# szcompressor/SZ3

Measured on AMD Instinct MI355X. Metric: compression throughput GB/s + ratio at fixed abs errBound, 512^3 f32, higher is better.
Workload: dtype f32; 1 GPU; C2: 3D float32 512x512x512 synthetic field per GPU, Lorenzo predictor, abs errBound=0.001, device-resident in -> device-resident Huffman payload; parallelism=slab1, algo=HIP_LORENZO(16), exchange=none (one rank)

## Files before the change

include/sz3hip_debug.h:

```cpp
#ifndef SZ3HIP_DEBUG_H
#define SZ3HIP_DEBUG_H

enum sz3hip_dbg {
    SZ3HIP_DBG_CB_COMPACT_IN_WG = 1,
    SZ3HIP_DBG_K1_LAB_NO_HIST = 1,
    SZ3HIP_DBG_DEC_MULTI_SYM = 2,
    SZ3HIP_DBG_K1_NO_CODE_STORES = 2,
    SZ3HIP_DBG_BLKDEC_FORCE_RETRY = 4,
    SZ3HIP_DBG_K1_V4_NO_STENCIL = 4,
    SZ3HIP_DBG_K1_NO_Q16 = 8,
    SZ3HIP_DBG_BLKDEC_LOCAL_EXPANDED = 16,
    SZ3HIP_DBG_K1_V4_NO_PREFETCH = 16,
    SZ3HIP_DBG_PACK_LAB_NO_STORES = 16,
    SZ3HIP_DBG_K1_NO_MARCH = 32,
    SZ3HIP_DBG_K1_NO_NARROW = 64,
    SZ3HIP_DBG_INTERP_NO_VEC = 128,
    SZ3HIP_DBG_K1_NO_WIDTH_SPEC = 256,
    SZ3HIP_DBG_DEC_NO_FUSED_X = 512,
    SZ3HIP_DBG_PACK_LAB_ONE_UNIT = 512,
    SZ3HIP_DBG_CB_ONE_CLASS = 1024,
    SZ3HIP_DBG_K1_NO_FUSED = 2048,
    SZ3HIP_DBG_BLK_RANK_3_LAUNCHES = 2048,
    SZ3HIP_DBG_BLK_SIDE_8_LAUNCHES = 2048,
    SZ3HIP_DBG_K1_NO_XCD_ORDER = 4096,
// ... 15 lines not shown
    SZ3HIP_DBG_K1_Q16_PLAIN_STORES = 8388608,
    SZ3HIP_DBG_K1_NO_DEFER_FOLD = 16777216,
    SZ3HIP_DBG_PACK_NO_SEG_BITS = 33554432,
    SZ3HIP_DBG_BLK_FIT_TILES = 67108864,
    SZ3HIP_DBG_BLK_1D_WAVE_PER_BLOCK = 134217728,
    SZ3HIP_DBG_CTX_NO_PUBLISH_ZERO = 268435456,
    SZ3HIP_DBG_INTERP_HANDOVER_IN_PLACE = 536870912,
    SZ3HIP_DBG_DEC_CARRY_PASS = 536870912,
    SZ3HIP_DBG_BLK_NO_EXIT = 1073741824,
    SZ3HIP_DBG_BLK_NO_SELECT = -2147483647 - 1
};

enum sz3hip_dbg2 {
    SZ3HIP_DBG2_PACK_SCAN_LAUNCH = 1,
    SZ3HIP_DBG2_REQUEST_BY_LEVEL = 2,
    SZ3HIP_DBG2_MAP_PLAIN_STORES = 4
};

#endif
```

sz3_amd/__init__.py:

```python
import contextlib
import ctypes as C
import enum
import os

import numpy as np

_HERE = os.path.dirname(os.path.abspath(__file__))
LIB_PATH = os.environ.get("SZ3HIP_LIB") or os.path.join(_HERE, "libsz3hip.so")

EB_ABS, EB_REL, EB_PSNR, EB_L2NORM, EB_ABS_AND_REL, EB_ABS_OR_REL = range(6)
ALGO_LORENZO_REG, ALGO_INTERP_LORENZO, ALGO_INTERP, ALGO_NOPRED, ALGO_LOSSLESS = range(5)
ALGO_HIP_LORENZO = 16
ALGO_HIP_INTERP = 17
INTERP_ALGO_LINEAR, INTERP_ALGO_CUBIC = 0, 1
SZ_FLOAT, SZ_DOUBLE = 0, 1


class Dbg(enum.IntFlag):
    CB_COMPACT_IN_WG = 1
    K1_LAB_NO_HIST = 1
    DEC_MULTI_SYM = 2
    K1_NO_CODE_STORES = 2
    BLKDEC_FORCE_RETRY = 4
    K1_V4_NO_STENCIL = 4
# ... 31 lines not shown
    K1_NO_DEFER_FOLD = 16777216
    PACK_NO_SEG_BITS = 33554432
    BLK_FIT_TILES = 67108864
    BLK_1D_WAVE_PER_BLOCK = 134217728
    CTX_NO_PUBLISH_ZERO = 268435456
    INTERP_HANDOVER_IN_PLACE = 536870912
    DEC_CARRY_PASS = 536870912
    BLK_NO_EXIT = 1073741824
    BLK_NO_SELECT = 2147483648


class Dbg2(enum.IntFlag):
    PACK_SCAN_LAUNCH = 1
    REQUEST_BY_LEVEL = 2
    MAP_PLAIN_STORES = 4


class SZ3HipError(RuntimeError):
    def __init__(self, code, msg):
        super().__init__("sz3hip error %d: %s" % (code, msg))
        self.code = code


class _CConfig(C.Structure):
    _fields_ = [
        ("N", C.c_int32), ("dims", C.c_uint64 * 4), ("num", C.c_uint64),
        ("cmprAlgo", C.c_uint8), ("errorBoundMode", C.c_uint8),
        ("absErrorBound", C.c_double), ("relErrorBound", C.c_double),
        ("psnrErrorBound", C.c_double), ("l2normErrorBound", C.c_double),
        ("openmp", C.c_uint8), ("quantbinCnt", C.c_int32), ("blockSize", C.c_int32),
# ... 1447 lines not shown
```

sz3_amd/csrc/sz3hip_kernels.h:

```cpp
#ifndef SZ3HIP_KERNELS_H
#define SZ3HIP_KERNELS_H
#include <hip/hip_runtime.h>
#include <stdint.h>
#include "sz3hip_format.h"
#include "../../include/sz3hip_debug.h"

struct szk_lattice {
    double recip, two_eb, eb;
    float recip_f, two_eb_f, eb_lo_f;
};
static inline szk_lattice szk_make_lattice(double eb) {
    szk_lattice l;
    l.eb = eb;
    l.two_eb = 2.0 * eb;
    l.recip = 1.0 / l.two_eb;
    l.recip_f = (float)l.recip;
    l.two_eb_f = (float)l.two_eb;
    float e = (float)eb;
    if ((double)e > eb) e = __builtin_nextafterf(e, 0.0f);
    l.eb_lo_f = e;
    return l;
}

#define SZK_K1_GRID 2048u
// ... 4 lines not shown
    uint32_t pack_wide;
    uint64_t n_samples;
    uint64_t n_total;
    uint32_t allow;
};

struct szk_cb_info;
#define SZK_SAMP_UNITS 1024u
#define SZK_SAMP_ROLES 128u
#define SZK_SAMP_MIN_ELEMS (1ull << 22)
#define SZK_SAMP_SEEN_LEN 16u
#define SZK_SAMP_WORDS 512u
#define SZK_SAMP_TICKET 320u
#define SZK_SAMP_LENS 384u
#define SZK_SAMP_READY 448u
struct szk_samp {
    uint32_t *words;
    uint32_t *enc;
    uint8_t *lens;
    szk_cb_info *info;
};
struct szk_k1_params {
    uint64_t d[4];
    szk_lattice lat;
    uint32_t radius;
    uint32_t dbg;
    szk_mode mode;
    uint64_t out_cap;
    uint64_t *hist;
    uint32_t *hist_partial;
// ... 14 lines not shown
    uint32_t *q16_flag;
    int defer_fold;
    uint32_t fold_rows;
    int range_kept;
    int fuse;
    int fused;
    const uint32_t *fuse_enc;
    const szk_cb_info *fuse_info;
    uint32_t *fuse_slots;
    uint64_t fuse_cap_words;
    uint32_t *seg_base;
    uint32_t *fuse_flag;
    uint32_t fuse_geom[4];
    szk_samp samp;
    int samp_in_launch;
};

struct szk_cb_info {
    uint32_t n_symbols, max_len, sym_min, sym_count;
    uint32_t win_lo, reserved;
    uint32_t esc_sym, pad0;
    uint64_t ts[12];
    uint32_t first_code[SZH_MAX_LEN + 2];
};
#define SZK_CB_DBG_ONE_CLASS 1u
#define SZK_CB_DBG_SERIAL_MERGE 2u
struct szk_cb_params {
    uint32_t *enc;
    uint8_t *lens;
    uint64_t *keys;
// ... 461 lines not shown
```

sz3_amd/csrc/sz3hip_kernels.hip:

```cpp
#include <hip/hip_runtime.h>
#include <cstddef>
#include <stdint.h>
#include <type_traits>
#include <mutex>
#include <utility>
#include <vector>
#include "sz3hip_format.h"
#include "sz3hip_kernels.h"

#include "sz3hip_devutil.h"

template <typename T>
__global__ __launch_bounds__(256) void k_minmax(const T *__restrict__ in, uint64_t n, double *partial) {
    double mn = INFINITY, mx = -INFINITY;
    bool has_nan = false;
    for (uint64_t i = (uint64_t)blockIdx.x * blockDim.x + threadIdx.x; i < n; i += (uint64_t)gridDim.x * blockDim.x) {
        double v = (double)in[i];
        if (v < mn) mn = v;
        if (v > mx) mx = v;
        has_nan |= (v != v);
    }
    (void)has_nan;
#pragma unroll
    for (int d = WAVE / 2; d > 0; d >>= 1) {
// ... 815 lines not shown
    uint16_t *seg_bits;
    uint64_t *oq_idx;
    OQV *oq_val;
    uint32_t oq_n;
    int lane;
    const uint32_t *s_enc;
    uint32_t *stage;
    uint32_t *slot;
    uint32_t slot_base;
    uint32_t slot_w;
    uint32_t st_cnt;
    uint32_t *seg_base;
    const uint32_t *samp_words;
    uint32_t *s_have;
    uint32_t have_len;
};
#define FUSE_STAGE_WORDS(TY) ((TY) * 128 + 32 + 8)
static inline uint32_t fuse_slot_words(uint32_t ty, uint64_t d1, uint64_t d2) {
    return (uint32_t)((d1 < ty ? d1 : ty) * 128u * (d2 < MARCH_TZ ? d2 : MARCH_TZ) + 32u);
}
template <typename T>
__device__ __forceinline__ void narrow_oq_flush(NarrowCtx<T> &c) {
    c.oq_n = (uint32_t)__builtin_amdgcn_readfirstlane((int)c.oq_n);
    if (c.oq_n == 0) return;
    const szk_k1_params &p = *c.p;
    const unsigned long long act = __ballot(1);
    const uint32_t nact = (uint32_t)__popcll(act), rank = (uint32_t)__popcll(act & ((1ull << c.lane) - 1ull));
    unsigned long long base = 0;
    if (rank == 0) base = atomicAdd((unsigned long long *)p.n_vout, (unsigned long long)c.oq_n);
    const uint32_t blo = (uint32_t)__builtin_amdgcn_readfirstlane((int)(uint32_t)base);
// ... 43 lines not shown
                c.oq_val[slot] = bits;
            }
            c.oq_n += (uint32_t)__popcll(vm);
        }
    }
    {
        const uint32_t cnt = (uint32_t)__popc(tmask & 15u);
        const unsigned long long b0 = __ballot(cnt & 1u), b1 = __ballot(cnt & 2u), b2 = __ballot(cnt & 4u), any = b0 | b1 | b2;
        if (any && c.lane == __ffsll((long long)any) - 1)
            hist_add_ranged(p.hist, p.range, 0u, (unsigned long long)(__popcll(b0) + 2 * __popcll(b1) + 4 * __popcll(b2)));
    }
}
template <typename T> __device__ __forceinline__ bool samp_take(const T *__restrict__ in, const szk_lattice &latp, uint32_t d0, uint32_t d1, uint32_t d2, uint32_t *words, uint32_t role, uint32_t *s_h);
__device__ __forceinline__ void samp_book(const szk_samp &sp, uint32_t radius, uint8_t *pool);
#define SAMP_POOL_BYTES (SZK_CB_SMALL_SYMS * 28 + 256)
template <typename T, typename PUT>
__device__ __forceinline__ bool samp_poll(NarrowCtx<T> &c, bool spin, PUT put) {
    volatile uint32_t *s_have = c.s_have;
    const uint32_t wv = (uint32_t)__builtin_amdgcn_readfirstlane((int)(threadIdx.x / WAVE));
    if (wv != 0) {
        uint32_t h = (uint32_t)__builtin_amdgcn_readfirstlane((int)*s_have);
        if (!h) {
            if (!spin) return false;
            do {
                __builtin_amdgcn_s_sleep(16);
                h = (uint32_t)__builtin_amdgcn_readfirstlane((int)*s_have);
            } while (!h);
        }
        __builtin_amdgcn_fence(__ATOMIC_ACQUIRE, "workgroup");
        c.have_len = 1;
// ... 102 lines not shown
#pragma unroll
            for (int r = 0; r <= TY; r++) {
                const uint32_t gy = y0 + (uint32_t)r - 1u;
                R.rok[lw][r] = wok && gy < d1;
                if (R.rok[lw][r]) {
                    const T *row = src + (uint64_t)gy * d0;
                    R.rq[lw][r].load(row + lane_off);
                    if (has_left) R.rl[lw][r] = row[x0 - 1];
                }
            }
        }
    };
    NarrowPlane<T, NW, TY> pa;
    auto work = [&](int zz, NarrowPlane<T, NW, TY> &R, bool fetch_next = false) {
        const uint32_t gz = z0 + (uint32_t)zz;
        if constexpr (FUSE) {
            __builtin_amdgcn_s_waitcnt(0x0F70);
            fuse_flush_lines(c);
        }
#if defined(LAB_MODE) && LAB_MODE == 1
        if (zz >= 0) {
#pragma unroll
            for (int r = 1; r <= TY; r++) {
                if (!R.rok[0][r]) continue;
                uint32_t acc = 0;
#pragma unroll
                for (int lw = 0; lw < NW; lw++)
#pragma unroll
                    for (int i = 0; i < 4; i++) acc += (uint32_t)lat.qbits(R.rq[lw][r].get(i)) + (has_left ? (uint32_t)lat.qbits(R.rl[lw][r]) : 0u);
                if (r == 1 && R.rok[0][0]) acc += (uint32_t)lat.qbits(R.rq[0][0].get(0));
// ... 80 lines not shown
#endif
                    const uint32_t l0 = e0 & 31u, l1 = e1 & 31u, l2 = e2 & 31u, l3 = e3 & 31u;
                    fp01[r - 1] = ((e0 >> 5) << l1) | (e1 >> 5);
                    fp23[r - 1] = ((e2 >> 5) << l3) | (e3 >> 5);
                    const uint32_t l23 = l2 + l3;
                    fl[r - 1] = (l0 + l1 + l23) | (l23 << 8);
                } else {
#ifdef LAB_ABLATE
                if (!(c.p->dbg & SZ3HIP_DBG_K1_NO_CODE_STORES))
#endif
#ifdef LAB_PLAIN_STORE
                *reinterpret_cast<uint32_t *>(c.codes8 + grow + x) = t[0] | (t[1] << 8) | (t[2] << 16) | (t[3] << 24);
#else
                __builtin_nontemporal_store(t[0] | (t[1] << 8) | (t[2] << 16) | (t[3] << 24), reinterpret_cast<uint32_t *>(c.codes8 + grow + x));
#endif
                }
            }
            if (SAMP ? c.have_len != 0u : c.s_len != nullptr) {
                uint32_t b4 = (uint32_t)c.s_len[t[0]] + c.s_len[t[1]] + c.s_len[t[2]] + c.s_len[t[3]];
                if (EDGE) b4 = xok ? b4 : 0u;
                bits_rows[(r - 1) >> 1] |= ((r - 1) & 1) ? b4 << 16 : b4;
            }
            if (__builtin_amdgcn_ballot_w64(rare)) {
                uint32_t tmask = 0, badmask = 0;
#pragma unroll
                for (int i = 0; i < 4; i++) {
                    tmask |= (uint32_t)(rare && t[i] == 255u) << i;
                    badmask |= (uint32_t)(rare && bad[i]) << i;
                }
                narrow_rare<T>(c, grow + x, delta, tmask, badmask);
// ... 86 lines not shown
                const uint32_t ra = y0 + 2u * k, rb = ra + 1u;
                if (lane == 0) {
                    const uint64_t g0 = (uint64_t)w * c.vol + (uint64_t)gz * c.plane + x0;
                    if (ra < d1) c.seg_bits[(g0 + (uint64_t)ra * d0) >> 8] = (uint16_t)(tot & 0xFFFFu);
                    if (2 * k + 1 < TY && rb < d1) c.seg_bits[(g0 + (uint64_t)rb * d0) >> 8] = (uint16_t)(tot >> 16);
                }
            }
        }
    };
    int zz = z0 > 0 ? -1 : 0;
    const int zend = d2 - z0 < (uint32_t)MARCH_TZ ? (int)(d2 - z0) : MARCH_TZ;
    if constexpr (SAMP) {
        uint8_t *const lt = const_cast<uint8_t *>(c.s_len);
        auto put_len = [&](uint32_t b, uint32_t len) { lt[b] = (uint8_t)len; };
        auto catch_up = [&](int zhi) __attribute__((always_inline)) {
            asm volatile("s_waitcnt vmcnt(0)" ::: "memory");
            constexpr int PB = 4;
            for (int p0 = 0; p0 < zhi; p0 += PB) {
                uint32_t cw[PB][TY];
#pragma unroll
                for (int j = 0; j < PB; j++) {
                    const uint64_t gp = (uint64_t)(z0 + (uint32_t)(p0 + j)) * c.plane;
#pragma unroll
                    for (int r = 0; r < TY; r++) {
                        const uint32_t ry = y0 + (uint32_t)r;
                        cw[j][r] = 0;
                        if (p0 + j < zhi && ry < d1 && xok)
                            cw[j][r] = __hip_atomic_load(reinterpret_cast<uint32_t *>(c.codes8 + gp + (uint64_t)ry * d0 + x), __ATOMIC_RELAXED, __HIP_MEMORY_SCOPE_WORKGROUP);
                    }
                }
#pragma unroll
                for (int j = 0; j < PB; j++) {
                    const uint64_t gp = (uint64_t)(z0 + (uint32_t)(p0 + j)) * c.plane;
                    if (p0 + j < zhi)
#pragma unroll
                    for (int k = 0; k < (TY + 1) / 2; k++) {
                        uint32_t packed = 0;
#pragma unroll
                        for (int h = 0; h < 2; h++) {
                            const uint32_t ry = y0 + 2u * k + h;
                            if (2 * k + h < TY && ry < d1 && xok) {
                                const uint32_t wd = cw[j][(2 * k + h) < TY ? 2 * k + h : 0];
                                const uint32_t b4 = (uint32_t)c.s_len[wd & 0xFFu] + c.s_len[(wd >> 8) & 0xFFu] + c.s_len[(wd >> 16) & 0xFFu] + c.s_len[wd >> 24];
// ... 35 lines not shown
        }
    } else if (FUSE) {
        fetch(zz, pa);
        for (; zz < zend; zz++) work(zz, pa, zz + 1 < zend);
    } else {
        for (; zz < zend; zz++) {
            fetch(zz, pa);
            work(zz, pa);
        }
    }
}
template <typename T, int NDIM, int TY, bool FUSE = false, bool SAMP = false>
__device__ __forceinline__ void march_narrow(const T *__restrict__ in, uint16_t *__restrict__ codes, const szk_k1_params &p, uint32_t ntasks,
                                             uint32_t *lh, uint8_t *s_len, uint64_t (*s_oq_idx)[MarchLds<1, false>::OQ],
                                             typename NarrowCtx<T>::OQV (*s_oq_val)[MarchLds<1, false>::OQ],
                                             uint32_t *s_fenc = nullptr, uint32_t *s_fstage = nullptr) {
    const Lattice<T> lat(p.lat);
    NarrowCtx<T> c;
    c.in = in;
    c.codes8 = reinterpret_cast<uint8_t *>(codes);
    c.p = &p;
    c.d0 = (uint32_t)p.d[3];
    c.d1 = (uint32_t)p.d[2];
    c.d2 = (uint32_t)p.d[1];
    c.plane = (uint64_t)c.d1 * c.d0;
    c.vol = c.plane * c.d2;
    c.lh = lh;
    c.lane = lane_id();
    const uint32_t wv = (uint32_t)__builtin_amdgcn_readfirstlane((int)(threadIdx.x / WAVE));
    c.oq_idx = s_oq_idx[wv];
    c.oq_val = s_oq_val[wv];
    c.oq_n = 0;
    const bool acct = SAMP || (!FUSE && p.spec_lens != nullptr && c.d0 % MARCH_TX == 0);
    c.s_len = acct ? s_len : nullptr;
    c.seg_bits = p.seg_bits;
    c.s_enc = s_fenc;
    c.stage = nullptr;
    c.slot = nullptr;
    c.slot_w = c.slot_base = c.st_cnt = 0;
    c.seg_base = p.seg_base;
    c.samp_words = p.samp.words;
    c.s_have = lh + NARROW_BINS * 4;
    c.have_len = 0;
    const uint32_t bid = SAMP ? blockIdx.x - SZK_SAMP_ROLES : blockIdx.x, grid = SAMP ? gridDim.x - SZK_SAMP_ROLES : gridDim.x;
    for (int i = threadIdx.x; i < NARROW_BINS * 4; i += 256) lh[i] = 0;
    if (threadIdx.x == 0) lh[NARROW_BINS * 4] = 0;
    if constexpr (FUSE) {
        const uint32_t ml = p.fuse_info->max_len, blo = p.fuse_info->sym_min, bcnt = p.fuse_info->sym_count;
        const uint32_t b = threadIdx.x;
        const uint32_t sym = b == 255u ? 0u : b + p.radius - 127u;
        s_fenc[b] = (ml <= 16u && sym >= blo && sym - blo < bcnt) ? p.fuse_enc[sym] : 0u;
        if (ml > 16u && blockIdx.x == 0 && threadIdx.x == 0) atomicOr(p.fuse_flag, 1u);
        for (int i = threadIdx.x; i < 4 * FUSE_STAGE_WORDS(TY); i += 256) s_fstage[i] = 0u;
        c.stage = s_fstage + wv * FUSE_STAGE_WORDS(TY);
        if (blockIdx.x == 0 && threadIdx.x == 0) *p.seg_made = 1u;
    }
    if (acct) {
        const uint32_t b = threadIdx.x;
// ... 105 lines not shown
#else
                R.rq[r] = *reinterpret_cast<const float4 *>(row + lane_off);
#endif
                if (has_left) R.rl[r] = row[x0 - 1];
            }
        }
    };
    Q16Plane<TY> pa;
    auto work = [&](int zz, Q16Plane<TY> &R) {
        const uint32_t gz = z0 + (uint32_t)zz;
        uint32_t pd1A = 0, pd1B = 0;
        uint32_t bits_rows[(TY + 1) / 2];
#pragma unroll
        for (int k = 0; k < (TY + 1) / 2; k++) bits_rows[k] = 0;
        float qmax = 0.0f;
#pragma unroll
        for (int r = 0; r <= TY; r++) {
            uint32_t d1A = 0, d1B = 0;
            v2f32 s01 = {0.0f, 0.0f}, s23 = {0.0f, 0.0f}, t01 = magic2, t23 = magic2;
            if (R.rok[r]) {
                const v2f32 v01 = {R.rq[r].x, R.rq[r].y}, v23 = {R.rq[r].z, R.rq[r].w};
                s01 = v01 * recip2;
                s23 = v23 * recip2;
                t01 = s01 + magic2;
                t23 = s23 + magic2;
                uint32_t PA = pk_lo16(__float_as_uint(t01.x), __float_as_uint(t23.x));
                uint32_t PB = pk_lo16(__float_as_uint(t01.y), __float_as_uint(t23.y));
                if (EDGE) {
                    PA = xok ? PA : 0u;
                    PB = xok ? PB : 0u;
// ... 34 lines not shown
                    atomicAdd(reinterpret_cast<uint32_t *>(lds + a0), 1u);
                    atomicAdd(reinterpret_cast<uint32_t *>(lds + a1), 1u);
                    atomicAdd(reinterpret_cast<uint32_t *>(lds + a2), 1u);
                    atomicAdd(reinterpret_cast<uint32_t *>(lds + a3), 1u);
                }
#if defined(LAB_ST) && LAB_ST == 1
                __hip_atomic_store(reinterpret_cast<uint32_t *>(c.codes8 + grow + x), tA | (tB << 8), __ATOMIC_RELAXED, __HIP_MEMORY_SCOPE_SYSTEM);
#elif defined(LAB_ST) && LAB_ST == 2
                *reinterpret_cast<uint32_t *>(c.codes8 + grow + x) = tA | (tB << 8);
#elif defined(LAB_ST) && LAB_ST == 3
                __hip_atomic_store(reinterpret_cast<uint32_t *>(c.codes8 + grow + x), tA | (tB << 8), __ATOMIC_RELAXED, __HIP_MEMORY_SCOPE_AGENT);
#else
                if (c.p->dbg & SZ3HIP_DBG_K1_Q16_PLAIN_STORES) *reinterpret_cast<uint32_t *>(c.codes8 + grow + x) = tA | (tB << 8);
                else __builtin_nontemporal_store(tA | (tB << 8), reinterpret_cast<uint32_t *>(c.codes8 + grow + x));
#endif
            }
            if (SAMP ? c.have_len != 0u : c.s_len != nullptr) {
                uint32_t b4 = (uint32_t)lds[Q16_LEN_OFF + a0] + lds[Q16_LEN_OFF + a1] + lds[Q16_LEN_OFF + a2] + lds[Q16_LEN_OFF + a3];
                if (EDGE) b4 = xok ? b4 : 0u;
                bits_rows[(r - 1) >> 1] |= ((r - 1) & 1) ? b4 << 16 : b4;
            }
            if (__builtin_amdgcn_ballot_w64(rare)) {
                const bool bad[4] = {b0, b1, b2, b3};
                const float sv[4] = {s01.x, s01.y, s23.x, s23.y};
                const uint32_t t[4] = {tA & 0xFFFFu, tB & 0xFFFFu, tA >> 16, tB >> 16};
                const uint32_t delta[4] = {(uint32_t)(int32_t)(int16_t)(sA & 0xFFFFu), (uint32_t)(int32_t)(int16_t)(sB & 0xFFFFu),
                                           (uint32_t)(int32_t)(int16_t)(sA >> 16), (uint32_t)(int32_t)(int16_t)(sB >> 16)};
                uint32_t tmask = 0, badmask = 0;
                bool alien = false;
#pragma unroll
// ... 21 lines not shown
                if (lane == 0) {
                    const uint64_t g0 = (uint64_t)gz * c.plane + x0;
                    if (ra < d1) c.seg_bits[(g0 + (uint64_t)ra * d0) >> 8] = (uint16_t)(tot & 0xFFFFu);
                    if (2 * k + 1 < TY && rb < d1) c.seg_bits[(g0 + (uint64_t)rb * d0) >> 8] = (uint16_t)(tot >> 16);
                }
            }
        }
    };
    int zz = z0 > 0 ? -1 : 0;
    const int zend = d2 - z0 < (uint32_t)MARCH_TZ ? (int)(d2 - z0) : MARCH_TZ;
    auto put_len = [&](uint32_t b, uint32_t len) {
        uint32_t *lt = c.lh + NARROW_BINS * 4 + b * 4u;
        lt[0] = lt[1] = lt[2] = lt[3] = len;
    };
    auto catch_up = [&](int zhi) __attribute__((always_inline)) {
        asm volatile("s_waitcnt vmcnt(0)" ::: "memory");
        constexpr int PB = 4;
        for (int p0 = 0; p0 < zhi; p0 += PB) {
            uint32_t cw[PB][TY];
#pragma unroll
            for (int j = 0; j < PB; j++) {
                const uint64_t gp = (uint64_t)(z0 + (uint32_t)(p0 + j)) * c.plane;
#pragma unroll
                for (int r = 0; r < TY; r++) {
                    const uint32_t ry = y0 + (uint32_t)r;
                    cw[j][r] = 0x80808080u;
                    if (p0 + j < zhi && ry < d1 && xok)
                        cw[j][r] = __hip_atomic_load(reinterpret_cast<uint32_t *>(c.codes8 + gp + (uint64_t)ry * d0 + x), __ATOMIC_RELAXED, __HIP_MEMORY_SCOPE_WORKGROUP);
                }
            }
#pragma unroll
            for (int j = 0; j < PB; j++) {
                const uint64_t gp = (uint64_t)(z0 + (uint32_t)(p0 + j)) * c.plane;
                if (p0 + j < zhi)
#pragma unroll
                for (int k = 0; k < (TY + 1) / 2; k++) {
                    uint32_t packed = 0;
#pragma unroll
                    for (int h = 0; h < 2; h++) {
                        const uint32_t ry = y0 + 2u * k + h;
                        if (2 * k + h < TY && ry < d1 && xok) {
                            const uint32_t w = cw[j][(2 * k + h) < TY ? 2 * k + h : 0];
                            const uint32_t b4 = (uint32_t)lds[Q16_LEN_OFF + (w & 0xFFu) * 16u + c4] + lds[Q16_LEN_OFF + ((w >> 8) & 0xFFu) * 16u + c4] +
// ... 32 lines not shown
        work(zz, pa);
        if (++zz >= zend) break;
        if (zz + 1 < zend) fetch(zz + 1, pa);
        work(zz, pb);
        if (++zz >= zend) break;
    }
#else
    for (; zz < zend; zz++) {
        fetch(zz, pa);
        work(zz, pa);
    }
#endif
}
template <int TY, bool SAMP>
__device__ __forceinline__ void march_narrow16(const float *__restrict__ in, uint16_t *__restrict__ codes, const szk_k1_params &p, uint32_t ntasks,
                                               uint32_t *lh, uint64_t (*s_oq_idx)[MarchLds<1, false>::OQ], uint32_t (*s_oq_val)[MarchLds<1, false>::OQ]) {
    const Lattice<float> lat(p.lat);
    NarrowCtx<float> c;
    c.in = in;
    c.codes8 = reinterpret_cast<uint8_t *>(codes);
    c.p = &p;
    c.d0 = (uint32_t)p.d[3];
    c.d1 = (uint32_t)p.d[2];
    c.d2 = (uint32_t)p.d[1];
    c.plane = (uint64_t)c.d1 * c.d0;
    c.vol = c.plane * c.d2;
    c.lh = lh;
    c.lane = lane_id();
    const uint32_t wv = (uint32_t)__builtin_amdgcn_readfirstlane((int)(threadIdx.x / WAVE));
    c.oq_idx = s_oq_idx[wv];
    c.oq_val = s_oq_val[wv];
    c.oq_n = 0;
    const bool acct = SAMP || (p.spec_lens != nullptr && c.d0 % MARCH_TX == 0);
    c.s_len = acct ? reinterpret_cast<const uint8_t *>(lh) + Q16_LEN_OFF : nullptr;
    c.seg_bits = p.seg_bits;
    c.s_enc = nullptr;
    c.stage = nullptr;
    c.slot = nullptr;
    c.slot_w = c.slot_base = c.st_cnt = 0;
    c.seg_base = p.seg_base;
    c.samp_words = p.samp.words;
    c.s_have = lh + NARROW_BINS * 8;
    c.have_len = 0;
    const uint32_t bid = SAMP ? blockIdx.x - SZK_SAMP_ROLES : blockIdx.x, grid = SAMP ? gridDim.x - SZK_SAMP_ROLES : gridDim.x;
    for (int i = threadIdx.x; i < NARROW_BINS * 4; i += 256) lh[i] = 0;
    if (threadIdx.x == 0) lh[NARROW_BINS * 8] = 0;
    {
        const uint32_t b = threadIdx.x;
        const uint32_t len = (acct && !SAMP) ? p.spec_lens[b == 255u ? 0u : b + p.radius - 127u] : 0u;
#pragma unroll
        for (int k = 0; k < 4; k++) lh[NARROW_BINS * 4 + b * 4 + k] = len;
        if (acct && bid == 0 && threadIdx.x == 0) *p.seg_made = 1u;
    }
    __syncthreads();
    const uint32_t ntx = (c.d0 + MARCH_TX - 1) / MARCH_TX, nty = (c.d1 + TY - 1) / TY;
    const uint32_t per_xcd = grid / 8u;
    const uint32_t wg_seq = grid % 8u == 0 && !(p.dbg & SZ3HIP_DBG_K1_NO_XCD_ORDER) ? (bid % 8u) * per_xcd + bid / 8u : bid;
    const uint32_t nwaves = grid * 4u;
// ... 49 lines not shown
    __shared__ uint64_t s_oq_idx[4][L::OQ];
    __shared__ OQV s_oq_val[4][L::OQ];
    __shared__ uint8_t s_len[256];
    __shared__ uint32_t s_p[4];
    if constexpr (SAMP) {
        static_assert(NDIM == 3, "1-D ... 3-D arrays");
        if (blockIdx.x < SZK_SAMP_ROLES) {
            if (blockIdx.x == 0 && threadIdx.x == 0) p.samp.info->ts[9] = wall_clock64();
            if (samp_take<T>(in, p.lat, (uint32_t)p.d[3], (uint32_t)p.d[2], (uint32_t)p.d[1], p.samp.words, blockIdx.x, lh)) samp_book(p.samp, p.radius, reinterpret_cast<uint8_t *>(lh));
            __syncthreads();
            probe_body<T, NDIM>(in, p, p.mode.n_total, p.mode.probe_big, s_p);
            return;
        }
    }
    probe_body<T, NDIM>(in, p, p.mode.n_total, p.mode.probe_big, s_p);
    march_narrow<T, NDIM, TY, false, SAMP>(in, codes, p, ntasks, lh, s_len, s_oq_idx, s_oq_val);
}
template <int TY, bool SAMP>
__global__ __launch_bounds__(256) void k_lorenzo_quant_march3q(const float *__restrict__ in, uint16_t *__restrict__ codes,
                                                               szk_k1_params p, uint32_t ntasks, uint32_t nrows) {
    using L = MarchLds<1, false>;
    __shared__ uint32_t lh[NARROW_BINS * 8 + 4];
    __shared__ uint64_t s_oq_idx[4][L::OQ];
    __shared__ uint32_t s_oq_val[4][L::OQ];
    __shared__ uint32_t s_p[4];
    if constexpr (SAMP) {
        static_assert(sizeof(lh) >= SAMP_POOL_BYTES && sizeof(lh) >= 4096, "the book's scratch fits the histogram");
        if (blockIdx.x < SZK_SAMP_ROLES) {
            if (blockIdx.x == 0 && threadIdx.x == 0) p.samp.info->ts[9] = wall_clock64();
            if (samp_take<float>(in, p.lat, (uint32_t)p.d[3], (uint32_t)p.d[2], (uint32_t)p.d[1], p.samp.words, blockIdx.x, lh)) samp_book(p.samp, p.radius, reinterpret_cast<uint8_t *>(lh));
            __syncthreads();
            probe_body<float, 3>(in, p, p.mode.n_total, p.mode.probe_big, s_p);
            return;
        }
    }
    probe_body<float, 3>(in, p, p.mode.n_total, p.mode.probe_big, s_p);
    march_narrow16<TY, SAMP>(in, codes, p, ntasks, lh, s_oq_idx, s_oq_val);
}
template <typename T, int NDIM, int TY>
__global__ __launch_bounds__(256) void k_lorenzo_quant_march3f(const T *__restrict__ in, uint16_t *__restrict__ codes,
                                                               szk_k1_params p, uint32_t ntasks, uint32_t nrows) {
    using L = MarchLds<1, false>;
    using OQV = typename std::conditional<sizeof(T) == 4, uint32_t, uint64_t>::type;
    __shared__ uint32_t lh[NARROW_BINS * 4 + 4];
    __shared__ uint64_t s_oq_idx[4][L::OQ];
    __shared__ OQV s_oq_val[4][L::OQ];
    __shared__ uint32_t s_p[4];
    __shared__ uint32_t s_fenc[256];
    __shared__ __align__(16) uint32_t s_fstage[4 * FUSE_STAGE_WORDS(TY)];
    probe_body<T, NDIM>(in, p, p.mode.n_total, p.mode.probe_big, s_p);
    march_narrow<T, NDIM, TY, true>(in, codes, p, ntasks, lh, nullptr, s_oq_idx, s_oq_val, s_fenc, s_fstage);
}
// ... 1187 lines not shown
    if (ln == 0) s_wc[wv] = (uint32_t)__popcll(pm);
    __syncthreads();
    uint32_t a = (uint32_t)__popcll(pm & lower);
    for (uint32_t k = 0; k < wv; k++) a += s_wc[k];
    const uint32_t m = s_wc[0] + s_wc[1] + s_wc[2] + s_wc[3];
    const uint64_t mykey = ((uint64_t)w << 16) | t;
    if (w) keys[a] = mykey;
    __syncthreads();
    uint32_t r = 0;
    if (w)
        for (uint32_t o = 0; o < m; o++) r += keys[o] < mykey;
    __syncthreads();
    if (w) keys[r] = mykey;
    __syncthreads();
    if (t == 0) sp.info->ts[3] = wall_clock64();
    if (t < WAVE) cb_merge_wave32(keys, reinterpret_cast<uint32_t *>(ifreq), pleaf, pint, m);
    __syncthreads();
    if (t == 0) sp.info->ts[4] = wall_clock64();
    for (uint32_t q = t; q + 1 < m; q += CB_THREADS) {
        if (q == m - 2) pint[q] = (uint16_t)q;
        aux[q] = q == m - 2 ? 0 : 1;
    }
    __syncthreads();
    for (uint32_t span = 1; span < m && span < 2 * L; span <<= 1) {
        for (uint32_t q = t; q + 1 < m; q += CB_THREADS) {
            const uint16_t j = pint[q];
            const uint32_t sum = (uint32_t)aux[q] + aux[j];
            aux2[q] = (uint16_t)(sum > 0xFFFFu ? 0xFFFFu : sum);
            pint2[q] = pint[j];
        }
        __syncthreads();
// ... 13 lines not shown
        pleaf[q] = (uint16_t)l;
        atomicAdd(&s_cnt[l], 1u);
    }
    __syncthreads();
    if (s_over) cb_kraft_repair(pleaf, m, s_cnt, L, CB_THREADS, kraft_ws);
    s_l[t] = 0;
    __syncthreads();
    for (uint32_t q = t; q < m; q += CB_THREADS) s_l[(uint32_t)(keys[q] & 0xFFFFu)] = (uint8_t)pleaf[q];
    __syncthreads();
    if (t == 0) sp.info->ts[8] = wall_clock64();
    uint32_t ubits = 0;
    while ((1u << ubits) < n_un) ubits++;
    const uint32_t len = (n_un == 0 || cnt != 0) ? s_l[t] : (uint32_t)s_l[rep] + ubits;
    __syncthreads();
    s_l[t] = (uint8_t)len;
    uint32_t rank = 0;
    for (uint32_t l = 1; l <= SZH_MAX_LEN; l++) {
        const unsigned long long lm = __ballot(len == l);
        if (ln == 0) s_lc[wv][l] = (uint32_t)__popcll(lm);
        if (len == l) rank = (uint32_t)__popcll(lm & lower);
    }
    __syncthreads();
    if (t == 0) {
        uint32_t code = 0, maxl = 0, prev = 0;
        for (uint32_t l = 1; l <= SZH_MAX_LEN; l++) {
            const uint32_t c = s_lc[0][l] + s_lc[1][l] + s_lc[2][l] + s_lc[3][l];
            code = (code + prev) << (l > 1 ? 1 : 0);
            s_first[l] = code;
            prev = c;
            if (c) maxl = l;
        }
        sp.info->n_symbols = 256;
        sp.info->max_len = maxl;
        sp.info->sym_min = lo;
        sp.info->sym_count = 256;
        sp.info->win_lo = lo;
        sp.info->reserved = 0;
        sp.info->esc_sym = esc;
    }
    __syncthreads();
    for (uint32_t k = 0; k < wv; k++) rank += s_lc[k][len];
    const uint32_t e = ((s_first[len] + rank) << 5) | len;
    sp.enc[lo + t] = e;
    sp.lens[lo + t] = (uint8_t)len;
    if (t == 255) sp.enc[0] = e;
    if (t < 64) {
        const uint32_t w4 = (uint32_t)s_l[4 * t] | ((uint32_t)s_l[4 * t + 1] << 8) | ((uint32_t)s_l[4 * t + 2] << 16) | ((uint32_t)s_l[4 * t + 3] << 24);
        __hip_atomic_store(&sp.words[SZK_SAMP_LENS + t], w4, __ATOMIC_RELAXED, __HIP_MEMORY_SCOPE_AGENT);
    }
    asm volatile("s_waitcnt vmcnt(0)" ::: "memory");
    __syncthreads();
    if (t == 0) {
        __hip_atomic_store(&sp.words[SZK_SAMP_READY], 1u, __ATOMIC_RELAXED, __HIP_MEMORY_SCOPE_AGENT);
        sp.info->ts[10] = wall_clock64();
    }
}

template <typename T>
__global__ __launch_bounds__(256) void k_sample(const T *__restrict__ in, szk_k1_params p) {
    __shared__ __align__(16) uint32_t s_pool[(SAMP_POOL_BYTES + 3) / 4 > 1024 ? (SAMP_POOL_BYTES + 3) / 4 : 1024];
    if (!szk_is_narrow(p.mode)) return;
    if (samp_take<T>(in, p.lat, (uint32_t)p.d[3], (uint32_t)p.d[2], (uint32_t)p.d[1], p.samp.words, blockIdx.x, s_pool)) samp_book(p.samp, p.radius, reinterpret_cast<uint8_t *>(s_pool));
}

__global__ __launch_bounds__(1024) void k_cb_compact(const uint64_t *__restrict__ hist, uint64_t *__restrict__ keys, uint16_t *__restrict__ syms,
                                                     uint64_t *__restrict__ part) {
    __shared__ uint32_t s_w[16], s_before, s_oct[48];
    __shared__ unsigned long long s_sum;
    const uint32_t t = threadIdx.x, lane = lane_id(), wv = t / WAVE, w = blockIdx.x;
    if (t == 0) {
// ... 2821 lines not shown
            if (nb > 0x7FFFFFFFull) return -1;
            hipLaunchKernelGGL((k_lorenzo_quant<T, 4, 64, 8, 4>), dim3((uint32_t)nb), dim3(256), 0, s, (const T *)d_in, codes, p);
            break;
    }
    SZK_CHECK_LAUNCH();
    return 0;
}
uint64_t szk_fuse_scratch_words(int ndim, const uint64_t d[4]) {
    if (ndim < 1 || ndim > 3 || d[3] % MARCH_TX != 0 || d[3] >= (1ull << 31) || d[2] >= (1ull << 31) || d[1] >= (1ull << 31)) return 0;
    const uint32_t ty = ndim == 1 ? 1u : (uint32_t)LAB_MTY;
    return march_tasks(d, ty) * fuse_slot_words(ty, d[2], d[1]) + 2;
}
int szk_launch_k1(int dtype, int ndim, const void *d_in, uint16_t *codes, szk_k1_params *p, hipStream_t s) {
    szk_k1_params &pp = *p;
    pp.dbg = (uint32_t)szk_dbg_flags;
    if (szk_dbg_flags & SZ3HIP_DBG_K1_NO_NARROW) pp.mode.allow = 0;
    return dtype == 0 ? launch_k1<float>(ndim, d_in, codes, pp, s) : launch_k1<double>(ndim, d_in, codes, pp, s);
}

int szk_launch_codebook(const uint64_t *d_hist, const szk_cb_params *p, hipStream_t s) {
    const uint32_t nb = p->n_books ? p->n_books : 1;
    szk_cb_params q = *p;
    q.n_books = nb;
    q.dbg = ((szk_dbg_flags & SZ3HIP_DBG_CB_ONE_CLASS) ? SZK_CB_DBG_ONE_CLASS : 0u) | ((szk_dbg_flags & SZ3HIP_DBG_CB_SERIAL_MERGE) ? SZK_CB_DBG_SERIAL_MERGE : 0u);
    if (nb > 1) {
        hipError_t e = hipMemsetAsync(q.range, 0, 16 * nb, s);
        if (e != hipSuccess) return (int)e;
    }
    if (!p->range_ready) hipLaunchKernelGGL(k_hist_range, dim3(SZH_HIST_BINS / 256, nb), dim3(256), 0, s, d_hist, q.range);
    q.keys_ready = nb == 1 && p->part_hint != 0 && !(szk_dbg_flags & SZ3HIP_DBG_CB_COMPACT_IN_WG) ? 1 : 0;
// ... 414 lines not shown
```

Before: 2520 GB/s.

## Stash early-plane codes in LDS for catch-up and publish sample lengths earlier

While the sampled codebook is not yet ready, the first few z-planes of quantized codes are also kept in a per-wave LDS stash. The catch-up pass that later builds histograms or lengths reads those planes from LDS instead of reloading them from global memory, and it skips the full vmcnt wait when every plane it needs is in the stash. Separately, the sample-codebook kernel now publishes code lengths and the ready flag before computing canonical codes, so marching blocks can start using lengths sooner. This costs extra LDS per workgroup, which a static_assert keeps within a five-workgroups-per-CU budget, and adds a per-store branch.

```diff
diff --git a/include/sz3hip_debug.h b/include/sz3hip_debug.h
--- a/include/sz3hip_debug.h
+++ b/include/sz3hip_debug.h
@@ -53,7 +53,8 @@
 enum sz3hip_dbg2 {
     SZ3HIP_DBG2_PACK_SCAN_LAUNCH = 1,
     SZ3HIP_DBG2_REQUEST_BY_LEVEL = 2,
-    SZ3HIP_DBG2_MAP_PLAIN_STORES = 4
+    SZ3HIP_DBG2_MAP_PLAIN_STORES = 4,
+    SZ3HIP_DBG2_K1_NO_STASH = 8
 };
 
 #endif
diff --git a/sz3_amd/__init__.py b/sz3_amd/__init__.py
--- a/sz3_amd/__init__.py
+++ b/sz3_amd/__init__.py
@@ -69,6 +69,7 @@
     PACK_SCAN_LAUNCH = 1
     REQUEST_BY_LEVEL = 2
     MAP_PLAIN_STORES = 4
+    K1_NO_STASH = 8
 
 
 class SZ3HipError(RuntimeError):
diff --git a/sz3_amd/csrc/sz3hip_kernels.h b/sz3_amd/csrc/sz3hip_kernels.h
--- a/sz3_amd/csrc/sz3hip_kernels.h
+++ b/sz3_amd/csrc/sz3hip_kernels.h
@@ -42,6 +42,7 @@
 #define SZK_SAMP_TICKET 320u
 #define SZK_SAMP_LENS 384u
 #define SZK_SAMP_READY 448u
+#define SZK_K1_STASH_PLANES 4
 struct szk_samp {
     uint32_t *words;
     uint32_t *enc;
@@ -86,6 +87,7 @@
     uint32_t fuse_geom[4];
     szk_samp samp;
     int samp_in_launch;
+    uint32_t stash_k;
 };
 
 struct szk_cb_info {
diff --git a/sz3_amd/csrc/sz3hip_kernels.hip b/sz3_amd/csrc/sz3hip_kernels.hip
--- a/sz3_amd/csrc/sz3hip_kernels.hip
+++ b/sz3_amd/csrc/sz3hip_kernels.hip
@@ -853,6 +853,8 @@
     const uint32_t *samp_words;
     uint32_t *s_have;
     uint32_t have_len;
+    uint32_t *stash;
+    uint32_t stash_k;
 };
 #define FUSE_STAGE_WORDS(TY) ((TY) * 128 + 32 + 8)
 static inline uint32_t fuse_slot_words(uint32_t ty, uint64_t d1, uint64_t d2) {
@@ -926,6 +928,7 @@
 template <typename T> __device__ __forceinline__ bool samp_take(const T *__restrict__ in, const szk_lattice &latp, uint32_t d0, uint32_t d1, uint32_t d2, uint32_t *words, uint32_t role, uint32_t *s_h);
 __device__ __forceinline__ void samp_book(const szk_samp &sp, uint32_t radius, uint8_t *pool);
 #define SAMP_POOL_BYTES (SZK_CB_SMALL_SYMS * 28 + 256)
+#define SAMP_BOOK_LDS_BYTES 1024
 template <typename T, typename PUT>
 __device__ __forceinline__ bool samp_poll(NarrowCtx<T> &c, bool spin, PUT put) {
     volatile uint32_t *s_have = c.s_have;
@@ -1058,6 +1061,7 @@
     NarrowPlane<T, NW, TY> pa;
     auto work = [&](int zz, NarrowPlane<T, NW, TY> &R, bool fetch_next = false) {
         const uint32_t gz = z0 + (uint32_t)zz;
+        const bool stashing = SAMP && !c.have_len && zz >= 0 && zz < (int)c.stash_k;
         if constexpr (FUSE) {
             __builtin_amdgcn_s_waitcnt(0x0F70);
             fuse_flush_lines(c);
@@ -1168,6 +1172,7 @@
 #else
                 __builtin_nontemporal_store(t[0] | (t[1] << 8) | (t[2] << 16) | (t[3] << 24), reinterpret_cast<uint32_t *>(c.codes8 + grow + x));
 #endif
+                if (SAMP && stashing) c.stash[(zz * TY + (r - 1)) * WAVE + lane] = t[0] | (t[1] << 8) | (t[2] << 16) | (t[3] << 24);
                 }
             }
             if (SAMP ? c.have_len != 0u : c.s_len != nullptr) {
@@ -1284,19 +1289,31 @@
         uint8_t *const lt = const_cast<uint8_t *>(c.s_len);
         auto put_len = [&](uint32_t b, uint32_t len) { lt[b] = (uint8_t)len; };
         auto catch_up = [&](int zhi) __attribute__((always_inline)) {
-            asm volatile("s_waitcnt vmcnt(0)" ::: "memory");
             constexpr int PB = 4;
+            static_assert(SZK_K1_STASH_PLANES % PB == 0, "a round's planes come all from the stash or all from memory");
+            const int ks = zhi < (int)c.stash_k ? zhi : (int)c.stash_k;
+            if (zhi > ks) asm volatile("s_waitcnt vmcnt(0)" ::: "memory");
             for (int p0 = 0; p0 < zhi; p0 += PB) {
                 uint32_t cw[PB][TY];
-#pragma unroll
-                for (int j = 0; j < PB; j++) {
-                    const uint64_t gp = (uint64_t)(z0 + (uint32_t)(p0 + j)) * c.plane;
-#pragma unroll
-                    for (int r = 0; r < TY; r++) {
-                        const uint32_t ry = y0 + (uint32_t)r;
-                        cw[j][r] = 0;
-                        if (p0 + j < zhi && ry < d1 && xok)
-                            cw[j][r] = __hip_atomic_load(reinterpret_cast<uint32_t *>(c.codes8 + gp + (uint64_t)ry * d0 + x), __ATOMIC_RELAXED, __HIP_MEMORY_SCOPE_WORKGROUP);
+                if (p0 < ks) {
+#pragma unroll
+                    for (int j = 0; j < PB; j++)
+#pragma unroll
+                        for (int r = 0; r < TY; r++) {
+                            cw[j][r] = 0;
+                            if (p0 + j < zhi && y0 + (uint32_t)r < d1 && xok) cw[j][r] = c.stash[((p0 + j) * TY + r) * WAVE + lane];
+                        }
+                } else {
+#pragma unroll
+                    for (int j = 0; j < PB; j++) {
+                        const uint64_t gp = (uint64_t)(z0 + (uint32_t)(p0 + j)) * c.plane;
+#pragma unroll
+                        for (int r = 0; r < TY; r++) {
+                            const uint32_t ry = y0 + (uint32_t)r;
+                            cw[j][r] = 0;
+                            if (p0 + j < zhi && ry < d1 && xok)
+                                cw[j][r] = __hip_atomic_load(reinterpret_cast<uint32_t *>(c.codes8 + gp + (uint64_t)ry * d0 + x), __ATOMIC_RELAXED, __HIP_MEMORY_SCOPE_WORKGROUP);
+                        }
                     }
                 }
 #pragma unroll
@@ -1362,7 +1379,7 @@
 __device__ __forceinline__ void march_narrow(const T *__restrict__ in, uint16_t *__restrict__ codes, const szk_k1_params &p, uint32_t ntasks,
                                              uint32_t *lh, uint8_t *s_len, uint64_t (*s_oq_idx)[MarchLds<1, false>::OQ],
                                              typename NarrowCtx<T>::OQV (*s_oq_val)[MarchLds<1, false>::OQ],
-                                             uint32_t *s_fenc = nullptr, uint32_t *s_fstage = nullptr) {
+                                             uint32_t *s_fenc = nullptr, uint32_t *s_fstage = nullptr, uint32_t *s_stash = nullptr) {
     const Lattice<T> lat(p.lat);
     NarrowCtx<T> c;
     c.in = in;
@@ -1390,6 +1407,8 @@
     c.samp_words = p.samp.words;
     c.s_have = lh + NARROW_BINS * 4;
     c.have_len = 0;
+    c.stash = SAMP ? s_stash + wv * (SZK_K1_STASH_PLANES * TY * WAVE) : nullptr;
+    c.stash_k = SAMP ? min(p.stash_k, (uint32_t)SZK_K1_STASH_PLANES) : 0u;
     const uint32_t bid = SAMP ? blockIdx.x - SZK_SAMP_ROLES : blockIdx.x, grid = SAMP ? gridDim.x - SZK_SAMP_ROLES : gridDim.x;
     for (int i = threadIdx.x; i < NARROW_BINS * 4; i += 256) lh[i] = 0;
     if (threadIdx.x == 0) lh[NARROW_BINS * 4] = 0;
@@ -1525,6 +1544,7 @@
 #pragma unroll
         for (int k = 0; k < (TY + 1) / 2; k++) bits_rows[k] = 0;
         float qmax = 0.0f;
+        const bool stashing = SAMP && !c.have_len && zz >= 0 && zz < (int)c.stash_k;
 #pragma unroll
         for (int r = 0; r <= TY; r++) {
             uint32_t d1A = 0, d1B = 0;
@@ -1589,6 +1609,7 @@
                 if (c.p->dbg & SZ3HIP_DBG_K1_Q16_PLAIN_STORES) *reinterpret_cast<uint32_t *>(c.codes8 + grow + x) = tA | (tB << 8);
                 else __builtin_nontemporal_store(tA | (tB << 8), reinterpret_cast<uint32_t *>(c.codes8 + grow + x));
 #endif
+                if (SAMP && stashing) c.stash[(zz * TY + (r - 1)) * WAVE + lane] = tA | (tB << 8);
             }
             if (SAMP ? c.have_len != 0u : c.s_len != nullptr) {
                 uint32_t b4 = (uint32_t)lds[Q16_LEN_OFF + a0] + lds[Q16_LEN_OFF + a1] + lds[Q16_LEN_OFF + a2] + lds[Q16_LEN_OFF + a3];
@@ -1640,19 +1661,31 @@
         lt[0] = lt[1] = lt[2] = lt[3] = len;
     };
     auto catch_up = [&](int zhi) __attribute__((always_inline)) {
-        asm volatile("s_waitcnt vmcnt(0)" ::: "memory");
         constexpr int PB = 4;
+        static_assert(SZK_K1_STASH_PLANES % PB == 0, "a round's planes come all from the stash or all from memory");
+        const int ks = zhi < (int)c.stash_k ? zhi : (int)c.stash_k;
+        if (zhi > ks) asm volatile("s_waitcnt vmcnt(0)" ::: "memory");
         for (int p0 = 0; p0 < zhi; p0 += PB) {
             uint32_t cw[PB][TY];
-#pragma unroll
-            for (int j = 0; j < PB; j++) {
-                const uint64_t gp = (uint64_t)(z0 + (uint32_t)(p0 + j)) * c.plane;
-#pragma unroll
-                for (int r = 0; r < TY; r++) {
-                    const uint32_t ry = y0 + (uint32_t)r;
-                    cw[j][r] = 0x80808080u;
-                    if (p0 + j < zhi && ry < d1 && xok)
-                        cw[j][r] = __hip_atomic_load(reinterpret_cast<uint32_t *>(c.codes8 + gp + (uint64_t)ry * d0 + x), __ATOMIC_RELAXED, __HIP_MEMORY_SCOPE_WORKGROUP);
+            if (p0 < ks) {
+#pragma unroll
+                for (int j = 0; j < PB; j++)
+#pragma unroll
+                    for (int r = 0; r < TY; r++) {
+                        cw[j][r] = 0x80808080u;
+                        if (p0 + j < zhi && y0 + (uint32_t)r < d1 && xok) cw[j][r] = c.stash[((p0 + j) * TY + r) * WAVE + lane];
+                    }
+            } else {
+#pragma unroll
+                for (int j = 0; j < PB; j++) {
+                    const uint64_t gp = (uint64_t)(z0 + (uint32_t)(p0 + j)) * c.plane;
+#pragma unroll
+                    for (int r = 0; r < TY; r++) {
+                        const uint32_t ry = y0 + (uint32_t)r;
+                        cw[j][r] = 0x80808080u;
+                        if (p0 + j < zhi && ry < d1 && xok)
+                            cw[j][r] = __hip_atomic_load(reinterpret_cast<uint32_t *>(c.codes8 + gp + (uint64_t)ry * d0 + x), __ATOMIC_RELAXED, __HIP_MEMORY_SCOPE_WORKGROUP);
+                    }
                 }
             }
 #pragma unroll
@@ -1715,7 +1748,8 @@
 }
 template <int TY, bool SAMP>
 __device__ __forceinline__ void march_narrow16(const float *__restrict__ in, uint16_t *__restrict__ codes, const szk_k1_params &p, uint32_t ntasks,
-                                               uint32_t *lh, uint64_t (*s_oq_idx)[MarchLds<1, false>::OQ], uint32_t (*s_oq_val)[MarchLds<1, false>::OQ]) {
+                                               uint32_t *lh, uint64_t (*s_oq_idx)[MarchLds<1, false>::OQ], uint32_t (*s_oq_val)[MarchLds<1, false>::OQ],
+                                               uint32_t *s_stash) {
     const Lattice<float> lat(p.lat);
     NarrowCtx<float> c;
     c.in = in;
@@ -1743,6 +1777,8 @@
     c.samp_words = p.samp.words;
     c.s_have = lh + NARROW_BINS * 8;
     c.have_len = 0;
+    c.stash = SAMP ? s_stash + wv * (SZK_K1_STASH_PLANES * TY * WAVE) : nullptr;
+    c.stash_k = SAMP ? min(p.stash_k, (uint32_t)SZK_K1_STASH_PLANES) : 0u;
     const uint32_t bid = SAMP ? blockIdx.x - SZK_SAMP_ROLES : blockIdx.x, grid = SAMP ? gridDim.x - SZK_SAMP_ROLES : gridDim.x;
     for (int i = threadIdx.x; i < NARROW_BINS * 4; i += 256) lh[i] = 0;
     if (threadIdx.x == 0) lh[NARROW_BINS * 8] = 0;
@@ -1822,7 +1858,13 @@
         }
     }
     probe_body<T, NDIM>(in, p, p.mode.n_total, p.mode.probe_big, s_p);
-    march_narrow<T, NDIM, TY, false, SAMP>(in, codes, p, ntasks, lh, s_len, s_oq_idx, s_oq_val);
+    if constexpr (SAMP) {
+        __shared__ uint32_t s_stash[4 * SZK_K1_STASH_PLANES * TY * WAVE];
+        static_assert(sizeof(lh) + sizeof(s_oq_idx) + sizeof(s_oq_val) + sizeof(s_len) + sizeof(s_p) + sizeof(s_stash) + SAMP_BOOK_LDS_BYTES <= 32768, "five workgroups per CU");
+        march_narrow<T, NDIM, TY, false, true>(in, codes, p, ntasks, lh, s_len, s_oq_idx, s_oq_val, nullptr, nullptr, s_stash);
+    } else {
+        march_narrow<T, NDIM, TY, false, false>(in, codes, p, ntasks, lh, s_len, s_oq_idx, s_oq_val);
+    }
 }
 template <int TY, bool SAMP>
 __global__ __launch_bounds__(256) void k_lorenzo_quant_march3q(const float *__restrict__ in, uint16_t *__restrict__ codes,
@@ -1843,7 +1885,13 @@
         }
     }
     probe_body<float, 3>(in, p, p.mode.n_total, p.mode.probe_big, s_p);
-    march_narrow16<TY, SAMP>(in, codes, p, ntasks, lh, s_oq_idx, s_oq_val);
+    if constexpr (SAMP) {
+        __shared__ uint32_t s_stash[4 * SZK_K1_STASH_PLANES * TY * WAVE];
+        static_assert(sizeof(lh) + sizeof(s_oq_idx) + sizeof(s_oq_val) + sizeof(s_p) + sizeof(s_stash) + SAMP_BOOK_LDS_BYTES <= 32768, "five workgroups per CU");
+        march_narrow16<TY, true>(in, codes, p, ntasks, lh, s_oq_idx, s_oq_val, s_stash);
+    } else {
+        march_narrow16<TY, false>(in, codes, p, ntasks, lh, s_oq_idx, s_oq_val, nullptr);
+    }
 }
 template <typename T, int NDIM, int TY>
 __global__ __launch_bounds__(256) void k_lorenzo_quant_march3f(const T *__restrict__ in, uint16_t *__restrict__ codes,
@@ -3061,7 +3109,16 @@
     if (w) keys[r] = mykey;
     __syncthreads();
     if (t == 0) sp.info->ts[3] = wall_clock64();
+#ifdef LAB_SAMP_MERGE_ROUNDS
+    {
+        uint32_t *nf32 = reinterpret_cast<uint32_t *>(ifreq), *lf32 = nf32 + CAP;
+        if (w) lf32[r] = w;
+        __syncthreads();
+        if (t < WAVE) cb_merge_rounds<true, true>(keys, ifreq, lf32, nf32, pleaf, pint, m, s_wc, WAVE);
+    }
+#else
     if (t < WAVE) cb_merge_wave32(keys, reinterpret_cast<uint32_t *>(ifreq), pleaf, pint, m);
+#endif
     __syncthreads();
     if (t == 0) sp.info->ts[4] = wall_clock64();
     for (uint32_t q = t; q + 1 < m; q += CB_THREADS) {
@@ -3105,6 +3162,17 @@
     const uint32_t len = (n_un == 0 || cnt != 0) ? s_l[t] : (uint32_t)s_l[rep] + ubits;
     __syncthreads();
     s_l[t] = (uint8_t)len;
+    __syncthreads();
+    if (t < 64) {
+        const uint32_t w4 = (uint32_t)s_l[4 * t] | ((uint32_t)s_l[4 * t + 1] << 8) | ((uint32_t)s_l[4 * t + 2] << 16) | ((uint32_t)s_l[4 * t + 3] << 24);
+        __hip_atomic_store(&sp.words[SZK_SAMP_LENS + t], w4, __ATOMIC_RELAXED, __HIP_MEMORY_SCOPE_AGENT);
+    }
+    asm volatile("s_waitcnt vmcnt(0)" ::: "memory");
+    __syncthreads();
+    if (t == 0) {
+        __hip_atomic_store(&sp.words[SZK_SAMP_READY], 1u, __ATOMIC_RELAXED, __HIP_MEMORY_SCOPE_AGENT);
+        sp.info->ts[10] = wall_clock64();
+    }
     uint32_t rank = 0;
     for (uint32_t l = 1; l <= SZH_MAX_LEN; l++) {
         const unsigned long long lm = __ballot(len == l);
@@ -3135,16 +3203,6 @@
     sp.enc[lo + t] = e;
     sp.lens[lo + t] = (uint8_t)len;
     if (t == 255) sp.enc[0] = e;
-    if (t < 64) {
-        const uint32_t w4 = (uint32_t)s_l[4 * t] | ((uint32_t)s_l[4 * t + 1] << 8) | ((uint32_t)s_l[4 * t + 2] << 16) | ((uint32_t)s_l[4 * t + 3] << 24);
-        __hip_atomic_store(&sp.words[SZK_SAMP_LENS + t], w4, __ATOMIC_RELAXED, __HIP_MEMORY_SCOPE_AGENT);
-    }
-    asm volatile("s_waitcnt vmcnt(0)" ::: "memory");
-    __syncthreads();
-    if (t == 0) {
-        __hip_atomic_store(&sp.words[SZK_SAMP_READY], 1u, __ATOMIC_RELAXED, __HIP_MEMORY_SCOPE_AGENT);
-        sp.info->ts[10] = wall_clock64();
-    }
 }
 
 template <typename T>
@@ -5996,6 +6054,7 @@
 int szk_launch_k1(int dtype, int ndim, const void *d_in, uint16_t *codes, szk_k1_params *p, hipStream_t s) {
     szk_k1_params &pp = *p;
     pp.dbg = (uint32_t)szk_dbg_flags;
+    pp.stash_k = (szk_dbg_flags2 & SZ3HIP_DBG2_K1_NO_STASH) ? 0u : (uint32_t)SZK_K1_STASH_PLANES;
     if (szk_dbg_flags & SZ3HIP_DBG_K1_NO_NARROW) pp.mode.allow = 0;
     return dtype == 0 ? launch_k1<float>(ndim, d_in, codes, pp, s) : launch_k1<double>(ndim, d_in, codes, pp, s);
 }
```

Result: no change. 2519 GB/s (-0.0%).
